# passcod/zarc

Measured on AMD Instinct MI355X. Metric: uncompressed GiB/s (pack) at zstd -3, higher is better.
Workload: dtype u8; 1 GPU; zarc pack 10000 x 1048576 B synthetic entries per GPU, zstd level 3, checksum on (BASELINE configs[1]); entries_per_gpu=10000, entries_total=10000, entry_bytes=1048576, level=3, kinds=text/records/lz/random round-robin

## Files before the change

include/zarc_gpu.h:

```cpp
#ifndef ZARC_GPU_H
#define ZARC_GPU_H
#include <stddef.h>
#include <stdint.h>

#ifdef __cplusplus
extern "C" {
#endif

#define ZARC_GPU_ABI_VERSION 2
#define ZARC_GPU_DIGEST_LEN 32
#define ZARC_GPU_ALIGN 16
#define ZARC_GPU_PAD 64

typedef struct zarc_gpu zarc_gpu_t;

enum {
    ZARC_GPU_OK = 0,
    ZARC_GPU_E_DEVICE = -1,
    ZARC_GPU_E_NOMEM = -2,
    ZARC_GPU_E_PARAM = -3,
    ZARC_GPU_E_UNSUPPORTED = -4,
    ZARC_GPU_E_DSTSIZE = -5,
    ZARC_GPU_E_CHECK = -6
};
// ... 22 lines not shown
    ZARC_GPU_P_ENABLE_LDM = 160,
    ZARC_GPU_P_LDM_HASH_LOG = 161,
    ZARC_GPU_P_LDM_MIN_MATCH = 162,
    ZARC_GPU_P_LDM_BUCKET_SIZE_LOG = 163,
    ZARC_GPU_P_LDM_HASH_RATE_LOG = 164,
    ZARC_GPU_P_CONTENT_SIZE_FLAG = 200,
    ZARC_GPU_P_CHECKSUM_FLAG = 201,
    ZARC_GPU_P_DICT_ID_FLAG = 202,
    ZARC_GPU_PX_SCRATCH_MB = 9001,
    ZARC_GPU_PX_STAGE_CHUNK = 9002,
    ZARC_GPU_PX_STAGE_THREAD = 9003,
    ZARC_GPU_PX_COPY_THREADS = 9004,
    ZARC_GPU_PX_DEC_GROUPS = 9005,
    ZARC_GPU_PX_ZERO_COPY = 9006,
    ZARC_GPU_PX_BLOCK_SPLIT = 9007,
    ZARC_GPU_PX_CHECK_FRAMES = 9008
};

typedef struct {
    int level;
    int checksum_flag;
    int content_size_flag;
    int window_log;
    int hash_log, chain_log, search_log, min_match, target_length, strategy;
    int compress;
} zarc_gpu_params;

int zarc_gpu_create(zarc_gpu_t **out, int device);
int zarc_gpu_device_count(void);
void zarc_gpu_destroy(zarc_gpu_t *h);
int zarc_gpu_set_parameter(zarc_gpu_t *h, int param_id, int value);
// ... 216 lines not shown
```

zarc_amd/_lib.py:

```python
import ctypes
import os

_HERE = os.path.dirname(os.path.abspath(__file__))
DEFAULT_LIB = os.path.join(_HERE, "libzarc_gpu.so")

ABI_VERSION = 2
DIGEST_LEN = 32
ALIGN = 16
PAD = 64

OK, E_DEVICE, E_NOMEM, E_PARAM, E_UNSUPPORTED, E_DSTSIZE, E_CHECK = 0, -1, -2, -3, -4, -5, -6
FRAME_OK, FRAME_CORRUPT, FRAME_CHECKSUM, FRAME_DIGEST, FRAME_DSTSIZE, FRAME_BAD_MAGIC, FRAME_UNSUPPORTED, FRAME_SRCSIZE, FRAME_DUPLICATE = range(9)
P_COMPRESSION_LEVEL, P_WINDOW_LOG, P_HASH_LOG, P_CHAIN_LOG, P_SEARCH_LOG, P_MIN_MATCH, P_TARGET_LENGTH, P_STRATEGY = 100, 101, 102, 103, 104, 105, 106, 107
P_ENABLE_LDM, P_LDM_HASH_LOG, P_LDM_MIN_MATCH, P_LDM_BUCKET_SIZE_LOG, P_LDM_HASH_RATE_LOG = 160, 161, 162, 163, 164
P_CONTENT_SIZE_FLAG, P_CHECKSUM_FLAG, P_DICT_ID_FLAG = 200, 201, 202
PX_SCRATCH_MB, PX_STAGE_CHUNK, PX_STAGE_THREAD, PX_COPY_THREADS, PX_DEC_GROUPS, PX_ZERO_COPY = 9001, 9002, 9003, 9004, 9005, 9006
PX_BLOCK_SPLIT = 9007
PX_CHECK_FRAMES = 9008
C_H2D, C_D2H, C_RING, C_DIRECT = range(4)
T_BLAKE3, T_XXH64, T_MATCH, T_ENTROPY, T_ASSEMBLE, T_DECODE, T_TOTAL, T_DEC_SEQS, T_DEC_LITS, T_DEC_FRAMES = range(10)
T_SEARCH = 10
T_LINES = 11
SEARCH_ICASE, SEARCH_MAX_PATTERN, SEARCH_NONE = 1, 256, 2 ** 64 - 1
SEARCH_MAX_SET = 1024
LINES_MAX_LINE = 65536
MATCH_FIXED, MATCH_SET, MATCH_REGEX = 0, 1, 2
SELECT_INVERT = 1
REGEX_MAX_PATTERN, REGEX_MAX_STATES = 1024, 64

EXPORTS = [
    "zarc_gpu_abi_version", "zarc_gpu_level_finder", "zarc_gpu_parameter_advisory", "zarc_gpu_device_count", "zarc_gpu_create", "zarc_gpu_destroy", "zarc_gpu_set_parameter", "zarc_gpu_get_params",
    "zarc_gpu_enable_compression", "zarc_gpu_bound", "zarc_gpu_error_name", "zarc_gpu_frame_status_name", "zarc_gpu_last_error",
    "zarc_gpu_pack_batch", "zarc_gpu_pack_batch_device", "zarc_gpu_pack_batch_dedup", "zarc_gpu_pack_batch_device_dedup", "zarc_gpu_unpack_batch", "zarc_gpu_unpack_batch_device",
# ... 160 lines not shown
```

zarc_amd/csrc/engine.hip:

```cpp
#include "../../include/zarc_gpu.h"
#include "zarc_kernels.h"
#include "zre_compile.h"
#include <algorithm>
#include <atomic>
#include <chrono>
#include <cstddef>
#include <cstdio>
#include <cstdlib>
#include <cstring>
#include <map>
#include <mutex>
#include <new>
#include <numeric>
#include <string>
#include <thread>
#include <vector>

namespace {

struct DevBuf {
    void *p = nullptr;
    size_t cap = 0;
    DevBuf() = default;
    DevBuf(const DevBuf &) = delete;
// ... 54 lines not shown
    hipEvent_t ev_g[DEC_GROUPS][12] = {};
    int dec_groups = 0;
    uint64_t dec_split_above = 0;
    float ms[ZARC_GPU_T_COUNT];
    size_t scratch_budget = 0;
    uint64_t stage_chunk = 0;
    int stage_thread = 1;
    int copy_threads = 8;
    uint8_t *meta_pin = nullptr;
    size_t meta_cap = 0, meta_used = 0;
    int ldm[5] = {0, 0, 0, 0, 0};
    DevBuf d_vout;
    DevBuf d_chk_off;
    DevBuf d_chk_order, d_chk_slices, d_chk_bad;
    int check_frames = 0;
    size_t chk_index = 0;
    uint32_t chk_at = 0;
    float chk_ms = 0;
    DevBuf d_vout2;
    DevBuf d_rp_order, d_rp_xxh;
    DevBuf d_srch_pat, d_srch_slices, d_srch_count, d_srch_first;
    DevBuf d_set, d_set_hits, d_set_which;
    ZarcSetDesc set_desc{};
    DevBuf d_regex, d_re_summary, d_re_entry;
    DevBuf d_ln_slices, d_ln_lines;
    DevBuf d_ln_base, d_ln_deliver;
    DevBuf d_ln_rec, d_ln_total, d_ln_text;
    DevBuf d_sel_slices, d_sel_count;
    DevBuf d_regex_fwd;
    DevBuf d_mt_bitoff, d_mt_bits;
// ... 320 lines not shown
        if (value < 0) return ZARC_GPU_E_PARAM;
        h->scratch_budget = (size_t)value << 20; return ZARC_GPU_OK;
    case ZARC_GPU_PX_STAGE_CHUNK:
        if (value != 0 && value < 4096) return ZARC_GPU_E_PARAM;
        h->stage_chunk = (uint64_t)value; return ZARC_GPU_OK;
    case ZARC_GPU_PX_STAGE_THREAD: h->stage_thread = value ? 1 : 0; return ZARC_GPU_OK;
    case ZARC_GPU_PX_COPY_THREADS:
        if (value < 1 || value > 64) return ZARC_GPU_E_PARAM;
        h->copy_threads = value; return ZARC_GPU_OK;
    case ZARC_GPU_PX_DEC_GROUPS:
        if (value < 0 || value > zarc_gpu::DEC_GROUPS) return ZARC_GPU_E_PARAM;
        h->dec_groups = value; return ZARC_GPU_OK;
    case ZARC_GPU_PX_ZERO_COPY: if (value < 0 || value > (1 << 20)) return ZARC_GPU_E_PARAM; h->zero_copy = value; return ZARC_GPU_OK;
    case ZARC_GPU_PX_BLOCK_SPLIT: if (value != 0 && value != 1) return ZARC_GPU_E_PARAM; h->block_split = value; return ZARC_GPU_OK;
    case ZARC_GPU_PX_CHECK_FRAMES: if (value != 0 && value != 1) return ZARC_GPU_E_PARAM; h->check_frames = value; return ZARC_GPU_OK;
    case ZARC_GPU_P_CONTENT_SIZE_FLAG:
        if (value != 1) return ZARC_GPU_E_UNSUPPORTED;
        return ZARC_GPU_OK;
    case ZARC_GPU_P_CHECKSUM_FLAG: h->params.checksum_flag = value ? 1 : 0; return ZARC_GPU_OK;
    case ZARC_GPU_P_DICT_ID_FLAG: return ZARC_GPU_OK;
    case ZARC_GPU_P_ENABLE_LDM: if (value < 0 || value > 2) return ZARC_GPU_E_PARAM; h->ldm[0] = value; return ZARC_GPU_OK;
    case ZARC_GPU_P_LDM_HASH_LOG: if (value != 0 && (value < 6 || value > 30)) return ZARC_GPU_E_PARAM; h->ldm[1] = value; return ZARC_GPU_OK;
    case ZARC_GPU_P_LDM_MIN_MATCH: if (value != 0 && (value < 4 || value > 4096)) return ZARC_GPU_E_PARAM; h->ldm[2] = value; return ZARC_GPU_OK;
    case ZARC_GPU_P_LDM_BUCKET_SIZE_LOG: if (value != 0 && (value < 1 || value > 8)) return ZARC_GPU_E_PARAM; h->ldm[3] = value; return ZARC_GPU_OK;
    case ZARC_GPU_P_LDM_HASH_RATE_LOG: if (value < 0 || value > 25) return ZARC_GPU_E_PARAM; h->ldm[4] = value; return ZARC_GPU_OK;
    default:
        if ((id >= 400 && id <= 402) || (id >= 500 && id <= 1020)) return ZARC_GPU_E_UNSUPPORTED;
        return ZARC_GPU_E_PARAM;
    }
}
// ... 371 lines not shown
                                       h->d_seq.as<uint64_t>(), h->d_lit.as<uint8_t>(), h->d_out.as<uint8_t>(), eprof, h->d_plan.as<ZgePlan>(),
                                       h->d_enc_err.as<uint32_t>(), h->d_zpieces.as<ZgePiece>());
                } else
                    hipLaunchKernelGGL(zarc_zge_entropy_split, dim3((unsigned)nb), dim3(64), 0, h->stream, (uint32_t)nb, slot, h->d_pblocks.as<ZgeBlock>(),
                                       h->d_seq.as<uint64_t>(), h->d_lit.as<uint8_t>(), h->d_out.as<uint8_t>(), eprof, h->d_zpieces.as<ZgePiece>());
            } else if (bp[1] - bp[0] > 1) {
                ZHIP(h->d_plan.reserve(nb * sizeof(ZgePlan)));
                std::vector<uint32_t> groups;
                for (size_t j = 0; j < m && bp[j + 1] - bp[j] > 1; j++)
                    for (uint64_t g0 = bp[j]; g0 < bp[j + 1]; g0 += ZGE_TABLE_GROUP) groups.push_back((uint32_t)g0);
                if ((rc = upload_u32(h, h->d_groups, groups.data(), groups.size()))) return rc;
                hipLaunchKernelGGL(zarc_zge_entropy_p1, dim3((unsigned)nb), dim3(64), 0, h->stream, (uint32_t)nb, slot, h->d_blocks.as<ZgeBlock>(),
                                   h->d_seq.as<uint64_t>(), h->d_lit.as<uint8_t>(), h->d_out.as<uint8_t>(), eprof, h->d_plan.as<ZgePlan>());
                hipLaunchKernelGGL(zarc_zge_plan, dim3((unsigned)groups.size()), dim3(64), 0, h->stream, (uint32_t)nb, h->d_blocks.as<ZgeBlock>(), h->d_plan.as<ZgePlan>(),
                                   h->d_groups.as<uint32_t>());
                hipLaunchKernelGGL(zarc_zge_entropy_p2, dim3((unsigned)nb), dim3(64), 0, h->stream, (uint32_t)nb, slot, h->d_blocks.as<ZgeBlock>(),
                                   h->d_seq.as<uint64_t>(), h->d_lit.as<uint8_t>(), h->d_out.as<uint8_t>(), eprof, h->d_plan.as<ZgePlan>(), h->d_enc_err.as<uint32_t>());
            } else
                hipLaunchKernelGGL(zarc_zge_entropy, dim3((unsigned)nb), dim3(64), 0, h->stream, (uint32_t)nb, slot, h->d_blocks.as<ZgeBlock>(),
                                   h->d_seq.as<uint64_t>(), h->d_lit.as<uint8_t>(), h->d_out.as<uint8_t>(), eprof);
        }
        ZHIP(hipGetLastError());
        ZHIP(t.mark(&c));
        if (!xxh_joined) { ZHIP(hipStreamWaitEvent(h->stream, h->ev_join, 0)); xxh_joined = true; }
        const uint64_t *const d_xxh = pl ? pl->d_xxh : h->d_xxh.as<uint64_t>();
        if (split)
            hipLaunchKernelGGL(zarc_zge_assemble_split, dim3((unsigned)m), dim3(256), 0, h->stream, P, base, d_off, d_len, h->d_order.as<uint32_t>(), (uint32_t)m,
                               h->d_block_prefix.as<uint64_t>(), h->d_blocks.as<ZgeBlock>(), h->d_out.as<uint8_t>(), d_xxh,
                               (uint8_t *)d_dst, h->d_dst_off.as<uint64_t>(), h->d_dst_len.as<uint64_t>(), h->d_pblocks.as<ZgeBlock>(), h->d_zpieces.as<ZgePiece>());
        else
// ... 1 lines not shown
                               h->d_block_prefix.as<uint64_t>(), h->d_blocks.as<ZgeBlock>(), h->d_out.as<uint8_t>(), d_xxh,
                               (uint8_t *)d_dst, h->d_dst_off.as<uint64_t>(), h->d_dst_len.as<uint64_t>());
        ZHIP(hipGetLastError());
        ZHIP(t.mark(&d));
        HOST_PHASE(3);
        ZHIP(hipStreamSynchronize(h->stream));
        HOST_PHASE(4);
        if (P.dbg & 1024) {
            unsigned long long prof[15];
            ZHIP(hipMemcpy(prof, (const char *)h->d_queue.p + 8, sizeof prof, hipMemcpyDeviceToHost));
            unsigned long long tot = 0;
            for (int i = 0; i < 15; i++) tot += prof[i];
            fprintf(stderr, "zge_match stage ticks (%% of %llu):", tot);
            for (int i = 0; i < 15; i++) fprintf(stderr, " %d:%.1f", i, tot ? 100.0 * (double)prof[i] / (double)tot : 0.0);
            fprintf(stderr, "\n");
            ZHIP(hipMemcpy(prof, (const char *)h->d_queue.p + 128, 6 * 8, hipMemcpyDeviceToHost));
            tot = 0;
            for (int i = 0; i < 6; i++) tot += prof[i];
            fprintf(stderr, "zge_entropy stage ticks (%% of %llu): hist %.1f huf-build %.1f lit-encode %.1f seq-prepass %.1f seq-tables %.1f seq-encode %.1f\n", tot,
                    100.0 * prof[0] / tot, 100.0 * prof[1] / tot, 100.0 * prof[2] / tot, 100.0 * prof[3] / tot, 100.0 * prof[4] / tot, 100.0 * prof[5] / tot);
        }
        ms_match += elapsed(h, a, b);
        ms_ent += elapsed(h, b, c);
        ms_asm += elapsed(h, c, d);
        t.next = 3;
        start = end;
    }
    if (!have_digests) ZHIP(hipStreamWaitEvent(h->stream, h->ev_join3, 0));
    ZHIP(hipMemcpyAsync(dst_len, h->d_dst_len.p, n * 8, hipMemcpyDeviceToHost, h->stream));
    if (!have_digests) ZHIP(hipMemcpyAsync(digest, h->d_digests.p, n * 32, hipMemcpyDeviceToHost, h->stream));
    uint32_t enc_err = 0;
    ZHIP(hipMemcpyAsync(&enc_err, h->d_enc_err.p, 4, hipMemcpyDeviceToHost, h->stream));
    ZHIP(hipStreamSynchronize(h->stream));
    if (enc_err) { set_error(h, "internal: a block the table plan guaranteed to end up compressed did not (its successor may repeat tables the decoder never saw)"); return ZARC_GPU_E_DEVICE; }
    if (status) for (size_t i = 0; i < n; i++) status[i] = ZARC_GPU_FRAME_OK;
// ... 2111 lines not shown
```

zarc_amd/csrc/zarc_kernels.h:

```cpp
#pragma once
#include <hip/hip_runtime.h>
#include <stdint.h>

enum {
    ZARC_FRAME_OK = 0, ZARC_FRAME_CORRUPT = 1, ZARC_FRAME_CHECKSUM = 2, ZARC_FRAME_DIGEST = 3,
    ZARC_FRAME_DSTSIZE = 4, ZARC_FRAME_BAD_MAGIC = 5, ZARC_FRAME_UNSUPPORTED = 6, ZARC_FRAME_SRCSIZE = 7
};

constexpr uint32_t ZARC_BLOCK_MAX = 128 * 1024;
constexpr uint32_t ZARC_BLOCK = 64 * 1024;
constexpr uint32_t ZARC_MAX_SEQ = ZARC_BLOCK / 3 + 8;

struct ZgeParams {
    int level, checksum, window_log, long_log, short_log, short_bytes, tile, sub, cap, min_match, min_rep, rep_search,
        back_cap, lazy, lazy_delta, lit_cost, match_cost, rep_cost, short_window_log, rep_back, tag_bits, seg_log,
        far_log, far_ways, far_step_log, far_res_log, far_short, far_skip, far_back, near16, far_cdc_log, far_min_frame, rep_pass, lazy2_delta, far_cap, cont_cap, ext_cap, live_reps, slot_bytes, dbg;
};
__host__ __device__ inline uint64_t zge_seq_stride(uint32_t slot_bytes) { return slot_bytes / 3 + 8; }
__host__ __device__ inline uint64_t zge_lit_stride(uint32_t slot_bytes) { return (uint64_t)slot_bytes + 64; }
__host__ __device__ inline uint64_t zge_out_stride(uint32_t slot_bytes) { return (uint64_t)slot_bytes + 1024; }
__host__ __device__ inline size_t zge_far_words(const ZgeParams &P) { return P.far_log ? (((size_t)P.far_ways << P.far_log) * (P.far_short ? 2 : 1)) : 0; }

struct ZgeBlock {
    uint32_t frame;
// ... 6 lines not shown
};
constexpr uint32_t ZGE_TABLE_GROUP = 16;
struct ZgePlanTable {
    int16_t norm[64];
    uint8_t desc[80];
    uint32_t count[64];
    uint32_t cost;
    uint8_t mode, al, nsym, dl, rle, pad[3];
};
struct ZgePlan {
    uint32_t active;
    uint32_t nseq;
    uint32_t lsz;
    uint32_t extra_bits;
    uint32_t guaranteed;
    uint32_t pad[3];
    ZgePlanTable t[3];
};
static_assert(sizeof(ZgePlanTable) == 476 && sizeof(ZgePlan) == 32 + 3 * 476, "plan record layout");
constexpr uint32_t ZGE_SPLIT_K = 16;
constexpr uint32_t ZGE_SPLIT_PIECE_COST = 192;
constexpr uint32_t ZGE_PIECE_UNUSED = 3;
struct ZgePiece {
    uint32_t seq_first;
    uint32_t lit_first;
    uint32_t src_off;
    uint32_t out_off;
    uint32_t out_cap;
    uint32_t pad[3];
};
__host__ __device__ inline uint64_t zge_pack_seq(uint32_t ll, uint32_t ml, uint32_t ofv) { return (uint64_t)ofv | ((uint64_t)ll << 28) | ((uint64_t)ml << 46); }
__host__ __device__ inline uint32_t zge_seq_ofv(uint64_t s) { return (uint32_t)(s & 0xFFFFFFFu); }
__host__ __device__ inline uint32_t zge_seq_ll(uint64_t s) { return (uint32_t)((s >> 28) & 0x3FFFFu); }
// ... 194 lines not shown
                               const uint32_t *order, const uint32_t *units , uint32_t n_units, const uint64_t *block_prefix, ZgeBlock *blocks,
                               uint64_t *seq_scratch, uint8_t *lit_scratch, uint32_t *queue, uint32_t *far_scratch);
__global__ void zarc_zge_match_deep(ZgeParams P, const uint8_t *src_base, const uint64_t *src_off, const uint64_t *src_len,
                                    const uint32_t *order, const uint32_t *units , uint32_t n_units, const uint64_t *block_prefix, ZgeBlock *blocks,
                                    uint64_t *seq_scratch, uint8_t *lit_scratch, uint32_t *queue, uint32_t *far_scratch);
#ifdef ZARC_GPU_DIAG
__global__ void zarc_zge_match_deep_diag(ZgeParams P, const uint8_t *src_base, const uint64_t *src_off, const uint64_t *src_len,
                                    const uint32_t *order, const uint32_t *units , uint32_t n_units, const uint64_t *block_prefix, ZgeBlock *blocks,
                                    uint64_t *seq_scratch, uint8_t *lit_scratch, uint32_t *queue, uint32_t *far_scratch);
#endif
__global__ void zarc_zge_entropy(uint32_t n_blocks, uint32_t slot_bytes, ZgeBlock *blocks, uint64_t *seq_scratch, const uint8_t *lit_scratch,
                                 uint8_t *out_scratch, unsigned long long *prof);
__global__ void zarc_zge_entropy_p1(uint32_t n_blocks, uint32_t slot_bytes, ZgeBlock *blocks, uint64_t *seq_scratch, const uint8_t *lit_scratch,
                                    uint8_t *out_scratch, unsigned long long *prof, ZgePlan *plans);
__global__ void zarc_zge_plan(uint32_t n_blocks, const ZgeBlock *blocks, ZgePlan *plans, const uint32_t *group_start);
__global__ void zarc_zge_entropy_p2(uint32_t n_blocks, uint32_t slot_bytes, ZgeBlock *blocks, uint64_t *seq_scratch, const uint8_t *lit_scratch,
                                    uint8_t *out_scratch, unsigned long long *prof, ZgePlan *plans, uint32_t *err);
__global__ void zarc_zge_assemble(ZgeParams P, const uint8_t *src_base, const uint64_t *src_off, const uint64_t *src_len,
                                  const uint32_t *order, uint32_t n_frames, const uint64_t *block_prefix, const ZgeBlock *blocks, const uint8_t *out_scratch,
                                  const uint64_t *xxh, uint8_t *dst_base, const uint64_t *dst_off, uint64_t *dst_len);
__global__ void zarc_zge_split(uint32_t n_blocks, uint32_t slot_bytes, const ZgeBlock *blocks, uint64_t *seq_scratch, const uint8_t *lit_scratch,
                               ZgeBlock *pblocks, ZgePiece *pieces);
__global__ void zarc_zge_entropy_split(uint32_t n_blocks, uint32_t slot_bytes, ZgeBlock *pblocks, uint64_t *seq_scratch, const uint8_t *lit_scratch,
                                       uint8_t *out_scratch, unsigned long long *prof, const ZgePiece *pieces);
__global__ void zarc_zge_entropy_p1_split(uint32_t n_blocks, uint32_t slot_bytes, ZgeBlock *pblocks, uint64_t *seq_scratch, const uint8_t *lit_scratch,
                                          uint8_t *out_scratch, unsigned long long *prof, ZgePlan *plans, const ZgePiece *pieces);
__global__ void zarc_zge_plan_split(uint32_t n_blocks, const ZgeBlock *blocks, ZgePlan *plans, const uint32_t *group_start, const ZgeBlock *pblocks);
__global__ void zarc_zge_entropy_p2_split(uint32_t n_blocks, uint32_t slot_bytes, ZgeBlock *pblocks, uint64_t *seq_scratch, const uint8_t *lit_scratch,
                                          uint8_t *out_scratch, unsigned long long *prof, ZgePlan *plans, uint32_t *err, const ZgePiece *pieces);
__global__ void zarc_zge_assemble_split(ZgeParams P, const uint8_t *src_base, const uint64_t *src_off, const uint64_t *src_len,
// ... 4 lines not shown
```

zarc_amd/csrc/zge_entropy.hip:

```cpp
#include "zarc_device.h"
#include "zarc_kernels.h"
#include "zge_seq_join.h"

namespace {

#ifdef ZARC_HIPEMU
#define ZGE_CLOCK() 0ull
#else
#define ZGE_CLOCK() ((unsigned long long)__builtin_readcyclecounter())
#endif
#define ENT_PROF(i) do { if (prof && lane == 0) { const unsigned long long now_ = ZGE_CLOCK(); atomicAdd(prof + (i), now_ - tprev); tprev = now_; } } while (0)

constexpr int HUF_MAXBITS = 11;
constexpr uint32_t MIN_HUF_LITERALS = 64;

__constant__ const int16_t E_LL_DEFAULT[36] = {4, 3, 2, 2, 2, 2, 2, 2, 2, 2, 2, 2, 2, 1, 1, 1, 2, 2,
                                               2, 2, 2, 2, 2, 2, 2, 3, 2, 1, 1, 1, 1, 1, -1, -1, -1, -1};
__constant__ const int16_t E_ML_DEFAULT[53] = {1, 4, 3, 2, 2, 2, 2, 2, 2, 1, 1, 1, 1, 1, 1, 1, 1, 1,
                                               1, 1, 1, 1, 1, 1, 1, 1, 1, 1, 1, 1, 1, 1, 1, 1, 1, 1,
                                               1, 1, 1, 1, 1, 1, 1, 1, 1, 1, -1, -1, -1, -1, -1, -1, -1};
__constant__ const int16_t E_OF_DEFAULT[29] = {1, 1, 1, 1, 1, 1, 2, 2, 2, 1, 1, 1, 1, 1, 1,
                                               1, 1, 1, 1, 1, 1, 1, 1, 1, -1, -1, -1, -1, -1};
__device__ __forceinline__ uint32_t ll_code(uint32_t ll)
{
// ... 106 lines not shown
    total = 0;
    for (int s = 0; s < nsym; s++) {
        const int n = norm[s];
        if (n == 0) { t.dnb[s] = ((al + 1) << 16) - T; t.dfs[s] = 0; continue; }
        if (n == -1 || n == 1) { t.dnb[s] = (al << 16) - T; t.dfs[s] = total - 1; total += 1; }
        else {
            const int max_bits_out = al - zd::hb32((uint32_t)(n - 1));
            const int min_state_plus = n << max_bits_out;
            t.dnb[s] = (max_bits_out << 16) - min_state_plus;
            t.dfs[s] = total - n;
            total += n;
        }
    }
    t.al = al;
}
__device__ void fse_build_ctab_wave(FseCtab &t, const int16_t *norm, int nsym, int al, uint8_t *cellsym, int lane)
{
    const int T = 1 << al, step = (T >> 1) + (T >> 3) + 3, mask = T - 1;
    const int n_l = lane < nsym ? (int)norm[lane] : 0;
    const uint32_t cells_l = n_l == -1 ? 1u : (uint32_t)n_l;
    const uint32_t reg_l = n_l > 0 ? (uint32_t)n_l : 0u;
    const uint32_t start_all = zd::wave_scan_incl(cells_l) - cells_l;
    const uint32_t start_reg = zd::wave_scan_incl(reg_l) - reg_l;
    const uint64_t lowm = zd::ballot(n_l == -1);
    const int nlow = (int)__popcll(lowm), high = T - 1 - nlow;
    if (n_l == -1) cellsym[T - 1 - (int)__popcll(lowm & ((1ull << lane) - 1))] = (uint8_t)lane;
    if (lane < nsym) { t.dfs[lane] = (int32_t)start_all; t.dnb[lane] = (int32_t)start_reg; }
    zd::wave_sync();
    {
        const int per = T >= 64 ? T / 64 : 1;
// ... 395 lines not shown
    unsigned long long tprev = ZGE_CLOCK();
    if (bi >= n_blocks) return;
    ZgeBlock *rec = blocks + bi;
    ZgePlan *const plan = PHASE ? plans + bi : nullptr;
    if (PHASE == 2 && !plan->active) return;
    if (rec->type == 1 || (SPLIT && rec->type == ZGE_PIECE_UNUSED)) { if (PHASE == 1 && lane == 0) plan->active = 0; return; }
    const uint32_t nlit = rec->nlit, src_len = rec->src_len;
    uint32_t nseq = PHASE == 2 ? plan->nseq : rec->nseq;
    const uint32_t slot_i = SPLIT ? bi / ZGE_SPLIT_K : bi;
    const uint32_t seq_first = SPLIT ? pieces[bi].seq_first : 0u, lit_first = SPLIT ? pieces[bi].lit_first : 0u;
    uint64_t *seq = seq_scratch + (uint64_t)slot_i * zge_seq_stride(slot_bytes) + seq_first;
    const uint8_t *lit = lit_scratch + (uint64_t)slot_i * zge_lit_stride(slot_bytes) + lit_first;
    uint8_t *out = out_scratch + (uint64_t)slot_i * zge_out_stride(slot_bytes) + (SPLIT ? pieces[bi].out_off : 0u);
    const uint32_t out_cap = SPLIT ? pieces[bi].out_cap : (uint32_t)zge_out_stride(slot_bytes);
    bool fail = false;

    uint32_t lsz = PHASE == 2 ? plan->lsz : 0u;
    if (PHASE != 2) {
        const uint32_t n = nlit;
        const uint32_t raw_hdr = n < 32 ? 1u : (n < 4096 ? 2u : 3u);
        for (int i = lane; i < 256; i += 64) L.h.count[i] = 0;
        zd::wave_sync();
        {
            const uint32_t n4 = n / 4;
            const uint32_t *l4 = (const uint32_t *)lit;
            for (uint32_t i0 = 0; i0 < n4; i0 += 256) {
                uint32_t wv[4];
#pragma unroll
                for (uint32_t k = 0; k < 4; k++) { const uint32_t i = i0 + 64 * k + (uint32_t)lane; wv[k] = i < n4 ? l4[i] : 0u; }
#pragma unroll
// ... 216 lines not shown
                pt->norm[lane] = L.s.norm[which][lane];
                pt->desc[lane] = L.s.desc[which][lane];
                if (lane < 16) pt->desc[64 + lane] = L.s.desc[which][64 + lane];
                if (lane == 0) {
                    pt->cost = (uint32_t)L.ctrl[X_COST_L + which];
                    pt->mode = (uint8_t)L.ctrl[X_MODE_L + which]; pt->al = (uint8_t)L.ctrl[X_AL_L + which]; pt->nsym = (uint8_t)L.ctrl[X_NSYM_L + which];
                    pt->dl = (uint8_t)L.ctrl[X_DL_L + which]; pt->rle = (uint8_t)L.ctrl[X_RLE_L + which];
                }
            }
            {
                uint32_t xb = 0;
                if (lane < 36) xb += L.s.cl[lane] * ll_code_bits((uint32_t)lane);
                if (lane < 53) xb += L.s.cm[lane] * ml_code_bits((uint32_t)lane);
                if (lane < 32) xb += L.s.co[lane] * (uint32_t)lane;
                xb = zd::wave_sum(xb);
                if (lane == 0) { plan->active = 1; plan->nseq = nseq; plan->lsz = lsz; plan->extra_bits = xb; plan->guaranteed = 0; }
            }
            return;
          }
          if (PHASE == 2) {
#pragma unroll
            for (int which = 0; which < 3; which++) {
                const ZgePlanTable *pt = &plan->t[which];
                L.s.norm[which][lane] = pt->norm[lane];
                L.s.desc[which][lane] = pt->desc[lane];
                if (lane < 16) L.s.desc[which][64 + lane] = pt->desc[64 + lane];
                if (lane == 0) {
                    L.ctrl[X_MODE_L + which] = pt->mode; L.ctrl[X_AL_L + which] = pt->al; L.ctrl[X_NSYM_L + which] = pt->nsym;
                    L.ctrl[X_DL_L + which] = pt->dl; L.ctrl[X_RLE_L + which] = pt->rle;
                }
            }
            zd::wave_sync();
          }
#pragma unroll
            for (int which = 0; which < 3; which++) {
                FseCtab tt = which == 0 ? FseCtab{L.s.st + ST_LL, L.s.dnb_ll, L.s.dfs_ll, 0}
                                        : (which == 1 ? FseCtab{L.s.st + ST_OF, L.s.dnb_of, L.s.dfs_of, 0} : FseCtab{L.s.st + ST_ML, L.s.dnb_ml, L.s.dfs_ml, 0});
                uint8_t *cells = (uint8_t *)L.s.pre;
                if (L.ctrl[X_MODE_L + which] != 1) fse_build_ctab_wave(tt, L.s.norm[which], L.ctrl[X_NSYM_L + which], L.ctrl[X_AL_L + which], cells, lane);
#ifdef ZGE_DEBUG_FSE
                if (L.ctrl[X_MODE_L + which] != 1 && lane == 0) {
                    static thread_local uint16_t st2[512]; static thread_local int32_t dnb2[64], dfs2[64]; static thread_local uint8_t cs2[512];
                    FseCtab t2 = {st2, dnb2, dfs2, 0};
                    const int nsym = L.ctrl[X_NSYM_L + which], al = L.ctrl[X_AL_L + which];
                    fse_build_ctab(t2, L.s.norm[which], nsym, al, cs2);
                    bool bad = false;
                    for (int i = 0; i < (1 << al); i++) bad |= st2[i] != tt.state_tab[i];
                    for (int i = 0; i < nsym; i++) bad |= dnb2[i] != tt.dnb[i] || dfs2[i] != tt.dfs[i];
                    if (bad) { for (int i = 0; i < (1 << al); i++) if (st2[i] != tt.state_tab[i]) { printf("st[%d] serial %d wave %d; ", i, st2[i], tt.state_tab[i]); break; }
                        for (int i = 0; i < nsym; i++) if (dnb2[i] != tt.dnb[i] || dfs2[i] != tt.dfs[i]) { printf("sym %d dnb %d/%d dfs %d/%d; ", i, dnb2[i], tt.dnb[i], dfs2[i], tt.dfs[i]); break; }
                        printf("FSE mismatch which %d al %d nsym %d mode %d:", which, al, nsym, L.ctrl[X_MODE_L + which]); for (int i = 0; i < nsym; i++) printf(" %d", L.s.norm[which][i]); printf("\n"); }
                }
#endif
            }
// ... 5 lines not shown
            if (pos + 4 + dl_l + dl_o + dl_m > scap) fail = true;
            if (!fail) {
                if (lane == 0) {
                    so[pos] = (uint8_t)((mode_l << 6) | (mode_o << 4) | (mode_m << 2));
                    uint32_t q = pos + 1;
                    if (mode_l == 1) so[q++] = (uint8_t)L.ctrl[X_RLE_L]; else for (uint32_t i = 0; i < dl_l; i++) so[q++] = L.s.desc[0][i];
                    if (mode_o == 1) so[q++] = (uint8_t)L.ctrl[X_RLE_O]; else for (uint32_t i = 0; i < dl_o; i++) so[q++] = L.s.desc[1][i];
                    if (mode_m == 1) so[q++] = (uint8_t)L.ctrl[X_RLE_M]; else for (uint32_t i = 0; i < dl_m; i++) so[q++] = L.s.desc[2][i];
                }
                pos += 1 + (mode_l == 1 ? 1u : dl_l) + (mode_o == 1 ? 1u : dl_o) + (mode_m == 1 ? 1u : dl_m);
                const int my_mode = lane == 0 ? mode_l : (lane == 1 ? mode_o : (lane == 2 ? mode_m : 1));
                uint32_t state = 0;
                WavePacker pk;
                pk.begin(L.stage, so + pos, scap - pos, lane);
                uint64_t s_next = (uint32_t)lane < nseq ? seq[nseq - 1 - (uint32_t)lane] : 0;
                for (uint32_t done = 0; done < nseq; done += 64) {
                    const uint32_t cnt = nseq - done < 64 ? nseq - done : 64;
                    uint32_t ll = 0, ml = 3, ofv = 1, llc = 0, mlc = 0, ofc = 0;
                    const uint64_t s = s_next;
                    if (done + 64 + (uint32_t)lane < nseq) s_next = seq[nseq - 1 - done - 64 - (uint32_t)lane];
                    if ((uint32_t)lane < cnt) {
                        ll = zge_seq_ll(s); ml = zge_seq_ml(s); ofv = zge_seq_ofv(s);
                        llc = ll_code(ll); mlc = ml_code(ml); ofc = (uint32_t)zd::hb32(ofv);
                        L.s.pre[0][lane] = (uint32_t)L.s.dnb_ll[llc] | ((uint64_t)(uint32_t)(2 * (L.s.dfs_ll[llc] + ST_LL)) << 32);
                        L.s.pre[1][lane] = (uint32_t)L.s.dnb_of[ofc] | ((uint64_t)(uint32_t)(2 * (L.s.dfs_of[ofc] + ST_OF)) << 32);
                        L.s.pre[2][lane] = (uint32_t)L.s.dnb_ml[mlc] | ((uint64_t)(uint32_t)(2 * (L.s.dfs_ml[mlc] + ST_ML)) << 32);
                    }
                    zd::wave_sync();
                    if (lane < 3 && my_mode != 1) {
                        uint64_t *const pp = L.s.pre[lane];
                        typedef uint16_t __attribute__((may_alias)) u16a;
                        typedef uint64_t __attribute__((may_alias)) u64a;
                        u16a *const sbp = (u16a *)&L.s.norm[0][0] + 64 * lane;
                        uint32_t e = 0;
                        if (done == 0) {
                            const uint64_t c0 = pp[0];
                            const int32_t d = (int32_t)(uint32_t)c0, f = (int32_t)(uint32_t)(c0 >> 32);
                            const int nb0 = (d + (1 << 15)) >> 16;
                            const int value = (nb0 << 16) - d;
                            state = *(const uint16_t *)((const uint8_t *)L.s.st + (2 * (value >> nb0) + f));
                            e = 1;
                        }
#define CHAIN_NEXT(cur) do { const uint32_t nb_ = (state + (uint32_t)(cur)) >> 16;                                     \
                             state = *(const uint16_t *)((const uint8_t *)L.s.st + ((int)((state >> nb_) << 1) + (int32_t)(uint32_t)((cur) >> 32))); } while (0)
// ... 4 lines not shown
                            CHAIN_NEXT(c0); four |= (uint64_t)state << 16;
                            CHAIN_NEXT(c1); four |= (uint64_t)state << 32;
                            CHAIN_NEXT(c2); four |= (uint64_t)state << 48;
                            CHAIN_NEXT(c3);
                            *(u64a *)(sbp + e) = four;
                        }
                        for (; e < cnt; e++) { const uint64_t c0 = pp[e]; sbp[e] = (uint16_t)state; CHAIN_NEXT(c0); }
#undef CHAIN_NEXT
                    }
                    zd::wave_sync();
                    uint64_t lo = 0;
                    uint32_t hi = 0, nb = 0;
                    if ((uint32_t)lane < cnt) {
                        uint32_t bo = 0, bm = 0, bl = 0;
                        const bool first = done + (uint32_t)lane == 0;
                        if (!first) {
                            if (mode_o != 1) { const uint32_t c = (uint32_t)L.s.pre[1][lane], sb = ((const uint16_t __attribute__((may_alias)) *)&L.s.norm[0][0])[1 * 64 + lane], n_ = (sb + c) >> 16; bo = (sb & ((1u << n_) - 1)) | (n_ << 16); }
                            if (mode_m != 1) { const uint32_t c = (uint32_t)L.s.pre[2][lane], sb = ((const uint16_t __attribute__((may_alias)) *)&L.s.norm[0][0])[2 * 64 + lane], n_ = (sb + c) >> 16; bm = (sb & ((1u << n_) - 1)) | (n_ << 16); }
                            if (mode_l != 1) { const uint32_t c = (uint32_t)L.s.pre[0][lane], sb = ((const uint16_t __attribute__((may_alias)) *)&L.s.norm[0][0])[0 * 64 + lane], n_ = (sb + c) >> 16; bl = (sb & ((1u << n_) - 1)) | (n_ << 16); }
                        }
                        uint64_t acc = bo & 0xFFFF; uint32_t sh = bo >> 16;
                        acc |= (uint64_t)(bm & 0xFFFF) << sh; sh += bm >> 16;
                        acc |= (uint64_t)(bl & 0xFFFF) << sh; sh += bl >> 16;
                        uint32_t xb;
                        acc |= (uint64_t)ll_extra(ll, llc, &xb) << sh; sh += xb;
                        acc |= (uint64_t)ml_extra(ml, mlc, &xb) << sh; sh += xb;
                        const uint64_t ofx = (uint64_t)(ofv - (1u << ofc));
                        lo = acc | (ofx << sh);
                        hi = sh == 0 ? 0u : (uint32_t)(ofx >> (64 - sh));
                        nb = sh + ofc;
                    }
                    pk.put(lo, hi, nb, lane);
                    zd::wave_sync();
                }
                {
                    const uint32_t st_l = zd::shfl(state, 0), st_o = zd::shfl(state, 1), st_m = zd::shfl(state, 2);
                    uint64_t lo = 0; uint32_t nb = 0;
                    if (lane == 0) {
                        if (mode_m != 1) { lo |= (uint64_t)(st_m & ((1u << al_m) - 1)) << nb; nb += (uint32_t)al_m; }
                        if (mode_o != 1) { lo |= (uint64_t)(st_o & ((1u << al_o) - 1)) << nb; nb += (uint32_t)al_o; }
                        if (mode_l != 1) { lo |= (uint64_t)(st_l & ((1u << al_l) - 1)) << nb; nb += (uint32_t)al_l; }
                    }
                    pk.put(lo, 0, nb, lane);
                }
                const uint32_t bytes = pk.finish(lane);
                if (pk.overflow || pos + bytes > scap) fail = true;
                ssz = pos + bytes;
            }
        }
    }
    ENT_PROF(5);
// ... 161 lines not shown
{
    __shared__ int16_t gnorm[3][64];
    __shared__ uint8_t gdesc[3][80];
    __shared__ uint32_t gdl[3];
    zge_plan_body<false>(gnorm, gdesc, gdl, n_blocks, blocks, plans, group_start, nullptr);
}
__global__ void __launch_bounds__(64) zarc_zge_plan_split(uint32_t n_blocks, const ZgeBlock *__restrict__ blocks, ZgePlan *__restrict__ plans,
                                                          const uint32_t *__restrict__ group_start, const ZgeBlock *__restrict__ pblocks)
{
    __shared__ int16_t gnorm[3][64];
    __shared__ uint8_t gdesc[3][80];
    __shared__ uint32_t gdl[3];
    zge_plan_body<true>(gnorm, gdesc, gdl, n_blocks, blocks, plans, group_start, pblocks);
}

#include "zge_split.hip"
```

Before: 44.53 GiB/s.

## Precompute FSE sequence states per table group in a dedicated kernel

Adds a zarc_zge_seq_states kernel that runs after planning. For runs of at least four blocks sharing repeat-mode FSE tables, it builds the encoding tables once and walks the serial FSE state chains for all blocks in parallel, one lane per block and table. The packed states are written into the literal scratch area, and entropy_p2 then skips its per-block table build and serial state prepass, computing only bit counts from the precomputed words. This trades an extra launch and scratch traffic for less serial work in the encode kernel; it is on by default.

```diff
diff --git a/include/zarc_gpu.h b/include/zarc_gpu.h
--- a/include/zarc_gpu.h
+++ b/include/zarc_gpu.h
@@ -60,7 +60,8 @@
     ZARC_GPU_PX_DEC_GROUPS = 9005,
     ZARC_GPU_PX_ZERO_COPY = 9006,
     ZARC_GPU_PX_BLOCK_SPLIT = 9007,
-    ZARC_GPU_PX_CHECK_FRAMES = 9008
+    ZARC_GPU_PX_CHECK_FRAMES = 9008,
+    ZARC_GPU_PX_SEQ_STATES = 9009
 };
 
 typedef struct {
diff --git a/zarc_amd/_lib.py b/zarc_amd/_lib.py
--- a/zarc_amd/_lib.py
+++ b/zarc_amd/_lib.py
@@ -17,6 +17,7 @@
 PX_SCRATCH_MB, PX_STAGE_CHUNK, PX_STAGE_THREAD, PX_COPY_THREADS, PX_DEC_GROUPS, PX_ZERO_COPY = 9001, 9002, 9003, 9004, 9005, 9006
 PX_BLOCK_SPLIT = 9007
 PX_CHECK_FRAMES = 9008
+PX_SEQ_STATES = 9009
 C_H2D, C_D2H, C_RING, C_DIRECT = range(4)
 T_BLAKE3, T_XXH64, T_MATCH, T_ENTROPY, T_ASSEMBLE, T_DECODE, T_TOTAL, T_DEC_SEQS, T_DEC_LITS, T_DEC_FRAMES = range(10)
 T_SEARCH = 10
diff --git a/zarc_amd/csrc/engine.hip b/zarc_amd/csrc/engine.hip
--- a/zarc_amd/csrc/engine.hip
+++ b/zarc_amd/csrc/engine.hip
@@ -92,6 +92,7 @@
     DevBuf d_chk_off;
     DevBuf d_chk_order, d_chk_slices, d_chk_bad;
     int check_frames = 0;
+    int seq_states = 1;
     size_t chk_index = 0;
     uint32_t chk_at = 0;
     float chk_ms = 0;
@@ -442,6 +443,7 @@
     case ZARC_GPU_PX_ZERO_COPY: if (value < 0 || value > (1 << 20)) return ZARC_GPU_E_PARAM; h->zero_copy = value; return ZARC_GPU_OK;
     case ZARC_GPU_PX_BLOCK_SPLIT: if (value != 0 && value != 1) return ZARC_GPU_E_PARAM; h->block_split = value; return ZARC_GPU_OK;
     case ZARC_GPU_PX_CHECK_FRAMES: if (value != 0 && value != 1) return ZARC_GPU_E_PARAM; h->check_frames = value; return ZARC_GPU_OK;
+    case ZARC_GPU_PX_SEQ_STATES: if (value < 0) return ZARC_GPU_E_PARAM; h->seq_states = value; return ZARC_GPU_OK;
     case ZARC_GPU_P_CONTENT_SIZE_FLAG:
         if (value != 1) return ZARC_GPU_E_UNSUPPORTED;
         return ZARC_GPU_OK;
@@ -843,6 +845,12 @@
                                    h->d_seq.as<uint64_t>(), h->d_lit.as<uint8_t>(), h->d_out.as<uint8_t>(), eprof, h->d_plan.as<ZgePlan>());
                 hipLaunchKernelGGL(zarc_zge_plan, dim3((unsigned)groups.size()), dim3(64), 0, h->stream, (uint32_t)nb, h->d_blocks.as<ZgeBlock>(), h->d_plan.as<ZgePlan>(),
                                    h->d_groups.as<uint32_t>());
+                if (h->seq_states) {
+                    uint32_t cap_words = (uint32_t)(zge_lit_stride(slot) / 4);
+                    if (h->seq_states > 1) cap_words = std::min<uint32_t>(cap_words, (uint32_t)h->seq_states);
+                    hipLaunchKernelGGL(zarc_zge_seq_states, dim3((unsigned)groups.size()), dim3(64), 0, h->stream, (uint32_t)nb, slot, h->d_blocks.as<ZgeBlock>(),
+                                       h->d_seq.as<uint64_t>(), h->d_lit.as<uint8_t>(), h->d_plan.as<ZgePlan>(), h->d_groups.as<uint32_t>(), cap_words, eprof);
+                }
                 hipLaunchKernelGGL(zarc_zge_entropy_p2, dim3((unsigned)nb), dim3(64), 0, h->stream, (uint32_t)nb, slot, h->d_blocks.as<ZgeBlock>(),
                                    h->d_seq.as<uint64_t>(), h->d_lit.as<uint8_t>(), h->d_out.as<uint8_t>(), eprof, h->d_plan.as<ZgePlan>(), h->d_enc_err.as<uint32_t>());
             } else
@@ -874,11 +882,12 @@
             fprintf(stderr, "zge_match stage ticks (%% of %llu):", tot);
             for (int i = 0; i < 15; i++) fprintf(stderr, " %d:%.1f", i, tot ? 100.0 * (double)prof[i] / (double)tot : 0.0);
             fprintf(stderr, "\n");
-            ZHIP(hipMemcpy(prof, (const char *)h->d_queue.p + 128, 6 * 8, hipMemcpyDeviceToHost));
+            ZHIP(hipMemcpy(prof, (const char *)h->d_queue.p + 128, 8 * 8, hipMemcpyDeviceToHost));
             tot = 0;
-            for (int i = 0; i < 6; i++) tot += prof[i];
-            fprintf(stderr, "zge_entropy stage ticks (%% of %llu): hist %.1f huf-build %.1f lit-encode %.1f seq-prepass %.1f seq-tables %.1f seq-encode %.1f\n", tot,
-                    100.0 * prof[0] / tot, 100.0 * prof[1] / tot, 100.0 * prof[2] / tot, 100.0 * prof[3] / tot, 100.0 * prof[4] / tot, 100.0 * prof[5] / tot);
+            for (int i = 0; i < 7; i++) tot += prof[i];
+            fprintf(stderr, "zge_entropy stage ticks (%% of %llu): hist %.1f huf-build %.1f lit-encode %.1f seq-prepass %.1f seq-tables %.1f seq-encode %.1f seq-states %.1f; seq-states blocks %llu\n", tot,
+                    100.0 * prof[0] / tot, 100.0 * prof[1] / tot, 100.0 * prof[2] / tot, 100.0 * prof[3] / tot, 100.0 * prof[4] / tot, 100.0 * prof[5] / tot,
+                    100.0 * prof[6] / tot, prof[7]);
         }
         ms_match += elapsed(h, a, b);
         ms_ent += elapsed(h, b, c);
diff --git a/zarc_amd/csrc/zarc_kernels.h b/zarc_amd/csrc/zarc_kernels.h
--- a/zarc_amd/csrc/zarc_kernels.h
+++ b/zarc_amd/csrc/zarc_kernels.h
@@ -44,9 +44,11 @@
     uint32_t lsz;
     uint32_t extra_bits;
     uint32_t guaranteed;
-    uint32_t pad[3];
+    uint32_t states;
+    uint32_t pad[2];
     ZgePlanTable t[3];
 };
+constexpr uint32_t ZGE_STATE_MIN_RUN = 4;
 static_assert(sizeof(ZgePlanTable) == 476 && sizeof(ZgePlan) == 32 + 3 * 476, "plan record layout");
 constexpr uint32_t ZGE_SPLIT_K = 16;
 constexpr uint32_t ZGE_SPLIT_PIECE_COST = 192;
@@ -271,6 +273,8 @@
 __global__ void zarc_zge_entropy_p1(uint32_t n_blocks, uint32_t slot_bytes, ZgeBlock *blocks, uint64_t *seq_scratch, const uint8_t *lit_scratch,
                                     uint8_t *out_scratch, unsigned long long *prof, ZgePlan *plans);
 __global__ void zarc_zge_plan(uint32_t n_blocks, const ZgeBlock *blocks, ZgePlan *plans, const uint32_t *group_start);
+__global__ void zarc_zge_seq_states(uint32_t n_blocks, uint32_t slot_bytes, const ZgeBlock *blocks, const uint64_t *seq_scratch, uint8_t *lit_scratch,
+                                    ZgePlan *plans, const uint32_t *group_start, uint32_t cap_words, unsigned long long *prof);
 __global__ void zarc_zge_entropy_p2(uint32_t n_blocks, uint32_t slot_bytes, ZgeBlock *blocks, uint64_t *seq_scratch, const uint8_t *lit_scratch,
                                     uint8_t *out_scratch, unsigned long long *prof, ZgePlan *plans, uint32_t *err);
 __global__ void zarc_zge_assemble(ZgeParams P, const uint8_t *src_base, const uint64_t *src_off, const uint64_t *src_len,
diff --git a/zarc_amd/csrc/zge_entropy.hip b/zarc_amd/csrc/zge_entropy.hip
--- a/zarc_amd/csrc/zge_entropy.hip
+++ b/zarc_amd/csrc/zge_entropy.hip
@@ -144,6 +144,14 @@
     }
     t.al = al;
 }
+__device__ __forceinline__ int32_t fse_sym_dnb(int n, int al)
+{
+    const int T = 1 << al;
+    if (n == 0) return ((al + 1) << 16) - T;
+    if (n == -1 || n == 1) return (al << 16) - T;
+    const int max_bits_out = al - zd::hb32((uint32_t)(n - 1));
+    return (max_bits_out << 16) - (n << max_bits_out);
+}
 __device__ void fse_build_ctab_wave(FseCtab &t, const int16_t *norm, int nsym, int al, uint8_t *cellsym, int lane)
 {
     const int T = 1 << al, step = (T >> 1) + (T >> 3) + 3, mask = T - 1;
@@ -569,6 +577,9 @@
     uint8_t *out = out_scratch + (uint64_t)slot_i * zge_out_stride(slot_bytes) + (SPLIT ? pieces[bi].out_off : 0u);
     const uint32_t out_cap = SPLIT ? pieces[bi].out_cap : (uint32_t)zge_out_stride(slot_bytes);
     bool fail = false;
+    constexpr bool STATES = PHASE == 2 && !SPLIT;
+    const bool given = STATES && plan->states != 0;
+    const uint32_t *const swords = (const uint32_t *)(lit_scratch + (uint64_t)slot_i * zge_lit_stride(slot_bytes));
 
     uint32_t lsz = PHASE == 2 ? plan->lsz : 0u;
     if (PHASE != 2) {
@@ -815,7 +826,7 @@
                 if (lane < 53) xb += L.s.cm[lane] * ml_code_bits((uint32_t)lane);
                 if (lane < 32) xb += L.s.co[lane] * (uint32_t)lane;
                 xb = zd::wave_sum(xb);
-                if (lane == 0) { plan->active = 1; plan->nseq = nseq; plan->lsz = lsz; plan->extra_bits = xb; plan->guaranteed = 0; }
+                if (lane == 0) { plan->active = 1; plan->nseq = nseq; plan->lsz = lsz; plan->extra_bits = xb; plan->guaranteed = 0; if (!SPLIT) plan->states = 0; }
             }
             return;
           }
@@ -838,7 +849,9 @@
                 FseCtab tt = which == 0 ? FseCtab{L.s.st + ST_LL, L.s.dnb_ll, L.s.dfs_ll, 0}
                                         : (which == 1 ? FseCtab{L.s.st + ST_OF, L.s.dnb_of, L.s.dfs_of, 0} : FseCtab{L.s.st + ST_ML, L.s.dnb_ml, L.s.dfs_ml, 0});
                 uint8_t *cells = (uint8_t *)L.s.pre;
-                if (L.ctrl[X_MODE_L + which] != 1) fse_build_ctab_wave(tt, L.s.norm[which], L.ctrl[X_NSYM_L + which], L.ctrl[X_AL_L + which], cells, lane);
+                if (STATES && given) {
+                    if (L.ctrl[X_MODE_L + which] != 1 && lane < L.ctrl[X_NSYM_L + which]) tt.dnb[lane] = fse_sym_dnb(L.s.norm[which][lane], L.ctrl[X_AL_L + which]);
+                } else if (L.ctrl[X_MODE_L + which] != 1) fse_build_ctab_wave(tt, L.s.norm[which], L.ctrl[X_NSYM_L + which], L.ctrl[X_AL_L + which], cells, lane);
 #ifdef ZGE_DEBUG_FSE
                 if (L.ctrl[X_MODE_L + which] != 1 && lane == 0) {
                     static thread_local uint16_t st2[512]; static thread_local int32_t dnb2[64], dfs2[64]; static thread_local uint8_t cs2[512];
@@ -874,20 +887,25 @@
                 WavePacker pk;
                 pk.begin(L.stage, so + pos, scap - pos, lane);
                 uint64_t s_next = (uint32_t)lane < nseq ? seq[nseq - 1 - (uint32_t)lane] : 0;
+                uint32_t w_next = STATES && given && (uint32_t)lane < nseq ? swords[nseq - 1 - (uint32_t)lane] : 0u;
                 for (uint32_t done = 0; done < nseq; done += 64) {
                     const uint32_t cnt = nseq - done < 64 ? nseq - done : 64;
                     uint32_t ll = 0, ml = 3, ofv = 1, llc = 0, mlc = 0, ofc = 0;
                     const uint64_t s = s_next;
+                    const uint32_t w = w_next;
                     if (done + 64 + (uint32_t)lane < nseq) s_next = seq[nseq - 1 - done - 64 - (uint32_t)lane];
+                    if (STATES && given && done + 64 + (uint32_t)lane < nseq) w_next = swords[nseq - 1 - done - 64 - (uint32_t)lane];
                     if ((uint32_t)lane < cnt) {
                         ll = zge_seq_ll(s); ml = zge_seq_ml(s); ofv = zge_seq_ofv(s);
                         llc = ll_code(ll); mlc = ml_code(ml); ofc = (uint32_t)zd::hb32(ofv);
+                      if (!(STATES && given)) {
                         L.s.pre[0][lane] = (uint32_t)L.s.dnb_ll[llc] | ((uint64_t)(uint32_t)(2 * (L.s.dfs_ll[llc] + ST_LL)) << 32);
                         L.s.pre[1][lane] = (uint32_t)L.s.dnb_of[ofc] | ((uint64_t)(uint32_t)(2 * (L.s.dfs_of[ofc] + ST_OF)) << 32);
                         L.s.pre[2][lane] = (uint32_t)L.s.dnb_ml[mlc] | ((uint64_t)(uint32_t)(2 * (L.s.dfs_ml[mlc] + ST_ML)) << 32);
+                      }
                     }
                     zd::wave_sync();
-                    if (lane < 3 && my_mode != 1) {
+                    if (lane < 3 && my_mode != 1 && !(STATES && given)) {
                         uint64_t *const pp = L.s.pre[lane];
                         typedef uint16_t __attribute__((may_alias)) u16a;
                         typedef uint64_t __attribute__((may_alias)) u64a;
@@ -922,7 +940,13 @@
                     if ((uint32_t)lane < cnt) {
                         uint32_t bo = 0, bm = 0, bl = 0;
                         const bool first = done + (uint32_t)lane == 0;
-                        if (!first) {
+                        if (STATES && given) {
+                            if (!first) {
+                                if (mode_o != 1) { const uint32_t c = (uint32_t)L.s.dnb_of[ofc], sb = (w >> 10) & 1023u, n_ = (sb + c) >> 16; bo = (sb & ((1u << n_) - 1)) | (n_ << 16); }
+                                if (mode_m != 1) { const uint32_t c = (uint32_t)L.s.dnb_ml[mlc], sb = w >> 20, n_ = (sb + c) >> 16; bm = (sb & ((1u << n_) - 1)) | (n_ << 16); }
+                                if (mode_l != 1) { const uint32_t c = (uint32_t)L.s.dnb_ll[llc], sb = w & 1023u, n_ = (sb + c) >> 16; bl = (sb & ((1u << n_) - 1)) | (n_ << 16); }
+                            }
+                        } else if (!first) {
                             if (mode_o != 1) { const uint32_t c = (uint32_t)L.s.pre[1][lane], sb = ((const uint16_t __attribute__((may_alias)) *)&L.s.norm[0][0])[1 * 64 + lane], n_ = (sb + c) >> 16; bo = (sb & ((1u << n_) - 1)) | (n_ << 16); }
                             if (mode_m != 1) { const uint32_t c = (uint32_t)L.s.pre[2][lane], sb = ((const uint16_t __attribute__((may_alias)) *)&L.s.norm[0][0])[2 * 64 + lane], n_ = (sb + c) >> 16; bm = (sb & ((1u << n_) - 1)) | (n_ << 16); }
                             if (mode_l != 1) { const uint32_t c = (uint32_t)L.s.pre[0][lane], sb = ((const uint16_t __attribute__((may_alias)) *)&L.s.norm[0][0])[0 * 64 + lane], n_ = (sb + c) >> 16; bl = (sb & ((1u << n_) - 1)) | (n_ << 16); }
@@ -942,7 +966,8 @@
                     zd::wave_sync();
                 }
                 {
-                    const uint32_t st_l = zd::shfl(state, 0), st_o = zd::shfl(state, 1), st_m = zd::shfl(state, 2);
+                    uint32_t st_l = zd::shfl(state, 0), st_o = zd::shfl(state, 1), st_m = zd::shfl(state, 2);
+                    if (STATES && given) { const uint32_t fin = swords[nseq]; st_l = fin & 1023u; st_o = (fin >> 10) & 1023u; st_m = fin >> 20; }
                     uint64_t lo = 0; uint32_t nb = 0;
                     if (lane == 0) {
                         if (mode_m != 1) { lo |= (uint64_t)(st_m & ((1u << al_m) - 1)) << nb; nb += (uint32_t)al_m; }
@@ -1134,4 +1159,147 @@
     zge_plan_body<true>(gnorm, gdesc, gdl, n_blocks, blocks, plans, group_start, pblocks);
 }
 
+namespace {
+constexpr int SS_ROW = 68;
+struct StatesLds {
+    alignas(16) uint32_t pre[3 * ZGE_TABLE_GROUP][SS_ROW];
+    uint16_t st[1280];
+    int32_t dnb_ll[36], dfs_ll[36], dnb_ml[53], dfs_ml[53], dnb_of[32], dfs_of[32];
+    uint32_t cc_ll[36], cc_of[32], cc_ml[53];
+    int16_t norm[3][64];
+    uint8_t cells[512];
+};
+}
+
+__global__ void __launch_bounds__(64) zarc_zge_seq_states(uint32_t n_blocks, uint32_t slot_bytes, const ZgeBlock *__restrict__ blocks, const uint64_t *__restrict__ seq_scratch,
+                                                          uint8_t *__restrict__ lit_scratch, ZgePlan *__restrict__ plans, const uint32_t *__restrict__ group_start,
+                                                          uint32_t cap_words, unsigned long long *__restrict__ prof )
+{
+    __shared__ StatesLds S;
+    const int lane = zd::lane_id();
+    const unsigned long long t_start = ZGE_CLOCK();
+    const uint32_t bi = group_start[blockIdx.x];
+    if (bi >= n_blocks) return;
+    const uint32_t frame = blocks[bi].frame, index0 = blocks[bi].index;
+    if (index0 % ZGE_TABLE_GROUP) return;
+    uint32_t nb = 1;
+    while (nb < ZGE_TABLE_GROUP && bi + nb < n_blocks && blocks[bi + nb].frame == frame && blocks[bi + nb].index == index0 + nb) nb++;
+    uint32_t act = 0, nsq = 0, m0 = 1, m1 = 1, m2 = 1;
+    if ((uint32_t)lane < nb) {
+        const ZgePlan *p = plans + bi + lane;
+        act = p->active; nsq = p->nseq; m0 = p->t[0].mode; m1 = p->t[1].mode; m2 = p->t[2].mode;
+    }
+    uint32_t prev_act = zd::shfl_up1(act);
+    if (lane == 0) prev_act = 0;
+    const bool cont = act && prev_act && (m0 == 1 || m0 == 3) && (m1 == 1 || m1 == 3) && (m2 == 1 || m2 == 3);
+    uint64_t heads = zd::ballot(act && !cont);
+    const uint64_t contm = zd::ballot(cont), fits = zd::ballot(act && nsq != 0 && nsq < cap_words);
+    uint32_t *const my_words = (uint32_t *)(lit_scratch + (uint64_t)(bi + ((uint32_t)lane < nb ? (uint32_t)lane : 0u)) * zge_lit_stride(slot_bytes));
+    while (heads) {
+        const uint32_t h = (uint32_t)zd::ctz64(heads);
+        heads &= heads - 1;
+        const uint32_t R = 1 + (uint32_t)zd::ctz64(~(contm >> (h + 1)));
+        const uint64_t taken = fits & (((1ull << R) - 1) << h);
+        if ((uint32_t)__popcll(taken) < ZGE_STATE_MIN_RUN) continue;
+        if (prof && lane == 0) atomicAdd(prof + 7, (unsigned long long)__popcll(taken));
+        const ZgePlan *const hp = plans + bi + h;
+        const int hm[3] = {(int)zd::readlane(m0, h), (int)zd::readlane(m1, h), (int)zd::readlane(m2, h)};
+#pragma unroll
+        for (int which = 0; which < 3; which++) S.norm[which][lane] = hp->t[which].norm[lane];
+        zd::wave_sync();
+#pragma unroll
+        for (int which = 0; which < 3; which++) {
+            FseCtab tt = which == 0 ? FseCtab{S.st + ST_LL, S.dnb_ll, S.dfs_ll, 0}
+                                    : (which == 1 ? FseCtab{S.st + ST_OF, S.dnb_of, S.dfs_of, 0} : FseCtab{S.st + ST_ML, S.dnb_ml, S.dfs_ml, 0});
+            const int nsym = hp->t[which].nsym, al = hp->t[which].al, nc = which == 0 ? 36 : (which == 1 ? 32 : 53);
+            uint32_t *const cc = which == 0 ? S.cc_ll : (which == 1 ? S.cc_of : S.cc_ml);
+            const int start = which == 0 ? ST_LL : (which == 1 ? ST_OF : ST_ML);
+            if (hm[which] != 1) fse_build_ctab_wave(tt, S.norm[which], nsym, al, S.cells, lane);
+            if (lane < nc) cc[lane] = hm[which] != 1 && lane < nsym ? (uint32_t)tt.dnb[lane] | ((uint32_t)(tt.dfs[lane] + start + 1024) << 20) : 1024u << 20;
+            zd::wave_sync();
+        }
+        const uint32_t cb = h + (uint32_t)lane / 3u, ct = (uint32_t)lane % 3u;
+        const uint32_t cb_c = cb < ZGE_TABLE_GROUP ? cb : 0u;
+        const uint32_t c_nseq = zd::shfl(nsq, (int)cb_c);
+        const uint32_t c_m0 = zd::shfl(m0, (int)cb_c), c_m1 = zd::shfl(m1, (int)cb_c), c_m2 = zd::shfl(m2, (int)cb_c);
+        const bool chain = (uint32_t)lane < 3 * R && ((taken >> cb_c) & 1) && (ct == 0 ? c_m0 : (ct == 1 ? c_m1 : c_m2)) != 1;
+        uint32_t state = 0;
+        const uint32_t maxn = zd::uniform(zd::wave_max(((taken >> lane) & 1) ? nsq : 0u));
+#define SS_EACH(X) X(0) X(1) X(2) X(3) X(4) X(5) X(6) X(7) X(8) X(9) X(10) X(11) X(12) X(13) X(14) X(15)
+#define SS_LOAD(r, at) { const bool on = (r) < R && ((taken >> (h + (r))) & 1); const uint32_t nr = on ? zd::readlane(nsq, h + (r)) : 0u, rb = on ? (r) : 0u;          \
+                         sv##r = seq_scratch[(uint64_t)(bi + h + rb) * zge_seq_stride(slot_bytes) + ((at) + (uint32_t)lane < nr ? nr - 1 - (at) - (uint32_t)lane : 0u)]; }
+#define SS_FIRST(r) uint64_t sv##r; SS_LOAD(r, 0u)
+        SS_EACH(SS_FIRST)
+#undef SS_FIRST
+        for (uint32_t done = 0; done < maxn; done += 64) {
+#define SS_POST(r) if ((r) < R && ((taken >> (h + (r))) & 1)) {                                                                                  \
+                const uint32_t nr = zd::readlane(nsq, h + (r));                                                                                 \
+                if (done < nr) {                                                                                                                \
+                    const uint64_t s = sv##r;                                                                                                   \
+                    if (done + (uint32_t)lane < nr) {                                                                                           \
+                        S.pre[3 * (r) + 0][lane] = S.cc_ll[ll_code(zge_seq_ll(s))];                                                             \
+                        S.pre[3 * (r) + 1][lane] = S.cc_of[zd::hb32(zge_seq_ofv(s))];                                                           \
+                        S.pre[3 * (r) + 2][lane] = S.cc_ml[ml_code(zge_seq_ml(s))];                                                             \
+                    } } }
+            SS_EACH(SS_POST)
+#undef SS_POST
+#define SS_AHEAD(r) SS_LOAD(r, done + 64)
+            SS_EACH(SS_AHEAD)
+#undef SS_AHEAD
+            zd::wave_sync();
+            if (chain && done < c_nseq) {
+                const uint32_t cnt = c_nseq - done < 64 ? c_nseq - done : 64;
+                uint32_t *const pp = S.pre[lane];
+                uint32_t e = 0;
+                if (done == 0) {
+                    const uint32_t c0 = pp[0];
+                    const int32_t d = (int32_t)(c0 & 0xFFFFFu);
+                    const int nb0 = (d + (1 << 15)) >> 16;
+                    const int value = (nb0 << 16) - d;
+                    state = *(const uint16_t *)((const uint8_t *)S.st + 2 * ((uint32_t)(value >> nb0) + (c0 >> 20)) - 2048);
+                    pp[0] = 0;
+                    e = 1;
+                }
+#define STATE_NEXT(cur) do { const uint32_t nb_ = (state + ((cur) & 0xFFFFFu)) >> 16;                                      \
+                             state = *(const uint16_t *)((const uint8_t *)S.st + 2 * ((state >> nb_) + ((cur) >> 20)) - 2048); } while (0)
+                for (; (e & 3u) && e < cnt; e++) { const uint32_t c0 = pp[e]; pp[e] = state; STATE_NEXT(c0); }
+                for (; e + 4 <= cnt; e += 4) {
+                    uint32_t c4[4], o4[4];
+                    __builtin_memcpy(c4, __builtin_assume_aligned(pp + e, 16), 16);
+                    o4[0] = state; STATE_NEXT(c4[0]);
+                    o4[1] = state; STATE_NEXT(c4[1]);
+                    o4[2] = state; STATE_NEXT(c4[2]);
+                    o4[3] = state; STATE_NEXT(c4[3]);
+                    __builtin_memcpy(__builtin_assume_aligned(pp + e, 16), o4, 16);
+                }
+                for (; e < cnt; e++) { const uint32_t c0 = pp[e]; pp[e] = state; STATE_NEXT(c0); }
+#undef STATE_NEXT
+            }
+            zd::wave_sync();
+#define SS_MERGE(r) if ((r) < R && ((taken >> (h + (r))) & 1)) {                                                                                 \
+                const uint32_t nr = zd::readlane(nsq, h + (r));                                                                                 \
+                if (done < nr) {                                                                                                                \
+                    const uint32_t k0 = zd::readlane(m0, h + (r)) != 1 ? 1023u : 0u, k1 = zd::readlane(m1, h + (r)) != 1 ? 1023u : 0u,           \
+                                   k2 = zd::readlane(m2, h + (r)) != 1 ? 1023u : 0u;                                                             \
+                    uint32_t *const words = (uint32_t *)(lit_scratch + (uint64_t)(bi + h + (r)) * zge_lit_stride(slot_bytes));                   \
+                    if (done + (uint32_t)lane < nr)                                                                                             \
+                        words[nr - 1 - done - (uint32_t)lane] = (S.pre[3 * (r) + 0][lane] & k0) | ((S.pre[3 * (r) + 1][lane] & k1) << 10) |     \
+                                                                 ((S.pre[3 * (r) + 2][lane] & k2) << 20);                                        \
+                } }
+            SS_EACH(SS_MERGE)
+#undef SS_MERGE
+            zd::wave_sync();
+        }
+#undef SS_LOAD
+#undef SS_EACH
+        {
+            const uint32_t rr = (uint32_t)lane >= h && (uint32_t)lane < h + R ? (uint32_t)lane - h : 0u;
+            const uint32_t fin = zd::shfl(state, (int)(3 * rr)) | (zd::shfl(state, (int)(3 * rr + 1)) << 10) | (zd::shfl(state, (int)(3 * rr + 2)) << 20);
+            if ((taken >> lane) & 1) { my_words[nsq] = fin; plans[bi + lane].states = 1; }
+        }
+        zd::wave_sync();
+    }
+    if (prof && lane == 0) atomicAdd(prof + 6, ZGE_CLOCK() - t_start);
+}
+
 #include "zge_split.hip"
```

Measured after the change: 45.66 GiB/s (median of 6 runs). 1.03x the previous value.
